# ReactiveBayes/RxInfer.jl

Measured on NVIDIA H100. Metric: gaussian_messages_per_sec_batched_lgssm_d4_T1000, higher is better.
Workload: dtype f32

## Files before the change

rxinfer.jl_b200/csrc/rxg_lgssm.cu:

```cuda
#include <math.h>
#include <stdlib.h>

#include <utility>

#include "rxg_chain_step.cuh"
#include "rxg_gain.cuh"
#include "rxg_internal.h"
#include "rxg_linalg.cuh"
#include "rxg_lgssm_cluster.cuh"
#include "rxg_lgssm_common.cuh"
#include "rxg_lgssm_shared.cuh"
#include "rxg_lgssm_seg.cuh"
#include "rxg_sweep_select.h"

namespace rxg {

template <int D, int M, bool PER_CHAIN, bool SMOOTH, bool USEQ = false>
__global__ void __launch_bounds__(128)
lgssm_chain_kernel(const __grid_constant__ ModelF<D, M> mdl, PerChainPtrs pc,
                   const float* __restrict__ y, const uint8_t* __restrict__ mask,
                   float* __restrict__ mean, float* __restrict__ cov, float* __restrict__ nle,
                   int32_t* __restrict__ status, int T, int64_t batch, int transition_first,
                   const float* __restrict__ useq = nullptr, int64_t ustride = 0, int uchain = 0) {
    const int64_t b = (int64_t)blockIdx.x * blockDim.x + threadIdx.x;
    if (b >= batch) return;

    Mat<float, D, D> A, P, S0;
    Mat<float, M, D> B;
    Mat<float, M, M> Q;
    Vec<float, D> mu, u;
    if (PER_CHAIN) {
        A = load_strided<float, D, D>(pc.A + b, batch);
        B = load_strided<float, M, D>(pc.B + b, batch);
        P = load_strided<float, D, D>(pc.P + b, batch);
        Q = load_strided<float, M, M>(pc.Q + b, batch);
        S0 = load_strided<float, D, D>(pc.S0 + b, batch);
#pragma unroll
        for (int i = 0; i < D; ++i) mu(i) = __ldg(pc.m0 + i * batch + b);
#pragma unroll
        for (int i = 0; i < D; ++i) u(i) = pc.u ? __ldg(pc.u + i * batch + b) : 0.f;
    } else {
        A = load_const<float, D, D>(mdl.A);
        B = load_const<float, M, D>(mdl.B);
        P = load_const<float, D, D>(mdl.P);
        Q = load_const<float, M, M>(mdl.Q);
        S0 = load_const<float, D, D>(mdl.S0);
#pragma unroll
        for (int i = 0; i < D; ++i) { mu(i) = mdl.m0[i]; u(i) = mdl.u[i]; }
    }
    Mat<float, D, D> S = S0;
    bool bad = false;
    double acc_nle = 0.0;
    const bool want_nle = (nle != nullptr);

    float ynext[M];
#pragma unroll
    for (int k = 0; k < M; ++k) ynext[k] = __ldg(y + (int64_t)k * batch + b);
    uint8_t onext = mask ? mask[b] : (uint8_t)1;

    for (int t = 0; t < T; ++t) {
        Vec<float, M> yt;
#pragma unroll
        for (int k = 0; k < M; ++k) yt(k) = ynext[k];
        const bool observed = onext != 0;
        if (t + 1 < T) {
#pragma unroll
            for (int k = 0; k < M; ++k) ynext[k] = __ldg(y + ((int64_t)(t + 1) * M + k) * batch + b);
            if (mask) onext = mask[(int64_t)(t + 1) * batch + b];
        }
        if (t > 0 || transition_first) {
            if constexpr (USEQ)
                chain_predict(A, P, u, [&](Vec<float, D>& uu) {
#pragma unroll
                    for (int i = 0; i < D; ++i) uu(i) = __ldg(useq + ((int64_t)t * D + i) * ustride + b * uchain);
                }, mu, S);
            else
                chain_predict(A, P, u, NoInput{}, mu, S);
        }
        if (observed) chain_update(B, Q, yt, want_nle, mu, S, bad, acc_nle);
#pragma unroll
        for (int i = 0; i < D; ++i) mean[((int64_t)t * D + i) * batch + b] = mu(i);
        const bool full = !SMOOTH || (t == T - 1);
#pragma unroll
        for (int i = 0; i < D; ++i)
#pragma unroll
            for (int j = 0; j < D; ++j)
                if (full || j <= i) cov[(((int64_t)t * D + i) * D + j) * batch + b] = S(i, j);
    }
    if (want_nle) nle[b] = (float)acc_nle;

    if (SMOOTH) {
        Vec<float, D> mus = mu;
        Mat<float, D, D> Ss = S;
        float pm[D], pS[D * (D + 1) / 2];
        if (T >= 2) {
            const int t = T - 2;
#pragma unroll
            for (int i = 0; i < D; ++i) pm[i] = mean[((int64_t)t * D + i) * batch + b];
            int q = 0;
#pragma unroll
            for (int i = 0; i < D; ++i)
#pragma unroll
                for (int j = 0; j <= i; ++j) pS[q++] = cov[(((int64_t)t * D + i) * D + j) * batch + b];
        }
        for (int t = T - 2; t >= 0; --t) {
            Vec<float, D> muf;
            Mat<float, D, D> Sf;
#pragma unroll
            for (int i = 0; i < D; ++i) muf(i) = pm[i];
            {
                int q = 0;
#pragma unroll
                for (int i = 0; i < D; ++i)
#pragma unroll
                    for (int j = 0; j <= i; ++j) { Sf(i, j) = pS[q]; Sf(j, i) = pS[q]; ++q; }
            }
            if (t > 0) {
                const int tp = t - 1;
#pragma unroll
                for (int i = 0; i < D; ++i) pm[i] = mean[((int64_t)tp * D + i) * batch + b];
                int q = 0;
#pragma unroll
                for (int i = 0; i < D; ++i)
#pragma unroll
                    for (int j = 0; j <= i; ++j) pS[q++] = cov[(((int64_t)tp * D + i) * D + j) * batch + b];
            }
            if constexpr (USEQ)
                chain_rts(A, P, u, [&](Vec<float, D>& uu) {
#pragma unroll
                    for (int i = 0; i < D; ++i) uu(i) = __ldg(useq + ((int64_t)(t + 1) * D + i) * ustride + b * uchain);
                }, muf, Sf, mus, Ss, bad);
            else
                chain_rts(A, P, u, NoInput{}, muf, Sf, mus, Ss, bad);
#pragma unroll
            for (int i = 0; i < D; ++i) mean[((int64_t)t * D + i) * batch + b] = mus(i);
#pragma unroll
            for (int i = 0; i < D; ++i)
#pragma unroll
                for (int j = 0; j < D; ++j) cov[(((int64_t)t * D + i) * D + j) * batch + b] = Ss(i, j);
        }
        mu = mus;
    }
    if (status) {
        bool nan = false;
#pragma unroll
        for (int i = 0; i < D; ++i) nan |= !(mu(i) == mu(i));
        status[b] = bad ? RXG_ERR_NOT_SPD : (nan ? RXG_ERR_NAN : RXG_OK);
    }
}

template <int D, int M>
__global__ void gain_riccati_seq(const __grid_constant__ ModelF<D, M> mdl, GainWs ws, int T,
                                 int transition_first, int* __restrict__ bad_out, const uint8_t* __restrict__ tmask) {
    if (threadIdx.x != 0 || blockIdx.x != 0) return;
    const Mat<double, D, D> A = load_const<double, D, D>(mdl.A), P = load_const<double, D, D>(mdl.P);
    const Mat<double, M, D> B = load_const<double, M, D>(mdl.B);
    const Mat<double, M, M> Q = load_const<double, M, M>(mdl.Q);
    Mat<double, D, D> S = load_const<double, D, D>(mdl.S0);
    bool bad = false;
    for (int t = 0; t < T; ++t) {
        if (t > 0 || transition_first) {
            Mat<double, D, D> AS = mul(A, S);
            S = sym_mul_nt_add(AS, A, P);
        }
        store_d(ws.Sp + (size_t)t * D * D, S);
        if (!tmask || tmask[t] != 0) {
            Mat<double, M, D> BS = mul(B, S);
            Mat<double, M, M> Sinn = sym_mul_nt_add(BS, B, Q);
            Chol<double, M> ch = cholesky<double, M, false>(Sinn, bad);
            Mat<double, D, M> V = solve_right_Lt(transpose(BS), ch.L);
            S = sym_downdate(S, V);
        }
        store_d(ws.Sf + (size_t)t * D * D, S);
    }
    if (bad) atomicOr(bad_out, 1);
}

template <int D, int M>
__global__ void gain_tables(const __grid_constant__ ModelF<D, M> mdl, GainWs ws, int T,
                            int transition_first, int* __restrict__ bad_out, const uint8_t* __restrict__ tmask,
                            const float* __restrict__ useq) {
    const int t = blockIdx.x * blockDim.x + threadIdx.x;
    if (t >= T) return;
    using TB = Tab<D, M>;
    const Mat<double, D, D> A = load_const<double, D, D>(mdl.A);
    const Mat<double, M, D> B = load_const<double, M, D>(mdl.B);
    const Mat<double, M, M> Q = load_const<double, M, M>(mdl.Q);
    bool bad = false;
    const Mat<double, D, D> Sp = load_d<D, D>(ws.Sp + (size_t)t * D * D);
    const Mat<double, D, D> Sf = load_d<D, D>(ws.Sf + (size_t)t * D * D);
    {
        Mat<double, D, M> K;
        Mat<double, M, M> Li;
        double cconst = 0.0;
#pragma unroll
        for (int i = 0; i < D * M; ++i) K.a[i] = 0.0;
#pragma unroll
        for (int i = 0; i < M * M; ++i) Li.a[i] = 0.0;
        if (!tmask || tmask[t] != 0) {
            Mat<double, M, D> BS = mul(B, Sp);
            Mat<double, M, M> Sinn = sym_mul_nt_add(BS, B, Q);
            Chol<double, M> ch = cholesky<double, M, true>(Sinn, bad);
            Mat<double, D, M> V = solve_right_Lt(transpose(BS), ch.L);
            K = solve_right_L(V, ch.L);
#pragma unroll
            for (int j = 0; j < M; ++j) {
                Li(j, j) = ch.L(j, j);
#pragma unroll
                for (int i = j + 1; i < M; ++i) {
                    double sacc = 0.0;
#pragma unroll
                    for (int k = j; k < i; ++k) sacc -= ch.L(i, k) * Li(k, j);
                    Li(i, j) = sacc * ch.L(i, i);
                }
            }
            cconst = M * RXG_HALF_LOG_2PI - ch.neg_half_logdet;
        }
        Mat<double, D, D> IKB = identity<double, D>();
#pragma unroll
        for (int i = 0; i < D; ++i)
#pragma unroll
            for (int j = 0; j < D; ++j)
#pragma unroll
                for (int k = 0; k < M; ++k) IKB(i, j) -= K(i, k) * B(k, j);
        Mat<double, D, D> F = (t > 0 || transition_first) ? mul(IKB, A) : IKB;
        float* rec = ws.fwd + (size_t)t * TB::FWD_REC;
        store_f(rec + TB::F_OFF, F);
        store_f(rec + TB::K_OFF, K);
        store_f(rec + TB::LI_OFF, Li);
        rec[TB::C_OFF] = (float)cconst;
        Vec<double, D> uu, gf;
#pragma unroll
        for (int i = 0; i < D; ++i) uu(i) = (double)(useq ? useq[(size_t)t * D + i] : mdl.u[i]);
        gf = mulv(IKB, uu);
        if (!(t > 0 || transition_first)) {
#pragma unroll
            for (int i = 0; i < D; ++i) gf(i) = 0.0;
        }
        store_fv(rec + TB::GF_OFF, gf);
        store_f(ws.sf + (size_t)t * TB::SF_REC, Sf);
    }
    float* brec = ws.bwd + (size_t)t * TB::BWD_REC;
    Vec<double, D> gb;
#pragma unroll
    for (int i = 0; i < D; ++i) gb(i) = 0.0;
    if (t < T - 1) {
        const Mat<double, D, D> Sp1 = load_d<D, D>(ws.Sp + (size_t)(t + 1) * D * D);
        Chol<double, D> ch = cholesky<double, D, false>(Sp1, bad);
        Mat<double, D, D> AS = mul(A, Sf);
        Mat<double, D, D> U = solve_right_Lt(transpose(AS), ch.L);
        Mat<double, D, D> G = solve_right_L(U, ch.L);
        Mat<double, D, D> C = sym_downdate(Sf, U);
        Mat<double, D, D> E = identity<double, D>();
        Mat<double, D, D> GA = mul(G, A);
#pragma unroll
        for (int i = 0; i < D * D; ++i) E.a[i] -= GA.a[i];
        store_f(brec + TB::E_OFF, E);
        store_f(brec + TB::G_OFF, G);
        {
            Vec<double, D> uu;
#pragma unroll
            for (int i = 0; i < D; ++i) uu(i) = -(double)(useq ? useq[(size_t)(t + 1) * D + i] : mdl.u[i]);
            gb = mulv(G, uu);
        }
        store_d(ws.Cc + (size_t)t * D * D, C);
        store_d(ws.Gd + (size_t)t * D * D, G);
    } else {
        Mat<double, D, D> E = identity<double, D>();
        Mat<double, D, D> Z;
#pragma unroll
        for (int i = 0; i < D * D; ++i) Z.a[i] = 0.0;
        store_f(brec + TB::E_OFF, E);
        store_f(brec + TB::G_OFF, Z);
    }
    store_fv(brec + TB::GB_OFF, gb);
    if (bad) atomicOr(bad_out, 1);
}

template <int D, int M>
__global__ void gain_smooth_seq(GainWs ws, int T, float* cov_shared_out) {
    if (threadIdx.x != 0 || blockIdx.x != 0) return;
    using TB = Tab<D, M>;
    Mat<double, D, D> Ss = load_d<D, D>(ws.Sf + (size_t)(T - 1) * D * D);
    store_f(ws.bwd + (size_t)(T - 1) * TB::BWD_REC + TB::SS_OFF, Ss);
    if (cov_shared_out) store_f(cov_shared_out + (size_t)(T - 1) * D * D, Ss);
    for (int t = T - 2; t >= 0; --t) {
        const Mat<double, D, D> G = load_d<D, D>(ws.Gd + (size_t)t * D * D);
        const Mat<double, D, D> C = load_d<D, D>(ws.Cc + (size_t)t * D * D);
        Mat<double, D, D> GS = mul(G, Ss);
        Ss = sym_mul_nt_add(GS, G, C);
        store_f(ws.bwd + (size_t)t * TB::BWD_REC + TB::SS_OFF, Ss);
        if (cov_shared_out) store_f(cov_shared_out + (size_t)t * D * D, Ss);
    }
}

static __global__ void copy_table_kernel(const float* __restrict__ tab, int rec, int n, int T, float* __restrict__ out) {
    const int i = blockIdx.x * blockDim.x + threadIdx.x;
    if (i < T * n) out[i] = tab[(size_t)(i / n) * rec + (i % n)];
}

template <int D, int M>
static void fill_model(ModelF<D, M>& mdl, const LgssmCall& c) {
    for (int i = 0; i < D * D; ++i) { mdl.A[i] = c.A[i]; mdl.P[i] = c.P[i]; mdl.S0[i] = c.S0[i]; }
    for (int i = 0; i < M * D; ++i) mdl.B[i] = c.B[i];
    for (int i = 0; i < M * M; ++i) mdl.Q[i] = c.Q[i];
    for (int i = 0; i < D; ++i) { mdl.m0[i] = c.m0[i]; mdl.u[i] = c.u ? c.u[i] : 0.f; }
}

template <int D, int M, bool PER_CHAIN, bool SMOOTH>
static void launch_chain(rxg_ctx* ctx, const LgssmCall& c, const ModelF<D, M>& mdl, const PerChainPtrs& pc) {
    const int threads = 64;
    const unsigned blocks = (unsigned)((c.batch + threads - 1) / threads);
    const int tf = (c.flags & RXG_TRANSITION_FIRST) ? 1 : 0;
    if (c.useq)
        lgssm_chain_kernel<D, M, PER_CHAIN, SMOOTH, true><<<blocks, threads, 0, ctx->stream>>>(
            mdl, pc, c.y, c.ymask, c.mean, c.cov, c.nle, c.status, c.T, c.batch, tf, c.useq, c.useq_chain ? c.batch : 1,
            c.useq_chain ? 1 : 0);
    else
        lgssm_chain_kernel<D, M, PER_CHAIN, SMOOTH><<<blocks, threads, 0, ctx->stream>>>(
            mdl, pc, c.y, c.ymask, c.mean, c.cov, c.nle, c.status, c.T, c.batch, tf);
}

template <int D, int M>
static int run_chain_family(rxg_ctx* ctx, LgssmCall& c) {
    ModelF<D, M> mdl = {};
    PerChainPtrs pc = {};
    const bool per_chain = (c.flags & RXG_MODEL_PER_CHAIN) != 0;
    if (per_chain) pc = PerChainPtrs{c.A, c.B, c.P, c.Q, c.m0, c.S0, c.u};
    else fill_model<D, M>(mdl, c);
    if (ctx->profile) { cudaEventRecord(ctx->ev[0], ctx->stream); cudaEventRecord(ctx->ev[1], ctx->stream); }
    if (per_chain) (c.smooth ? launch_chain<D, M, true, true> : launch_chain<D, M, true, false>)(ctx, c, mdl, pc);
    else           (c.smooth ? launch_chain<D, M, false, true> : launch_chain<D, M, false, false>)(ctx, c, mdl, pc);
    if (ctx->profile) cudaEventRecord(ctx->ev[2], ctx->stream);
    ctx->launches += 1;
    return check_cuda(ctx, cudaGetLastError(), "lgssm_chain_kernel launch");
}

template <int D, int M, int I>
static bool launch_sweep_if(int pick, rxg_ctx* ctx, const LgssmCall& c, const ModelF<D, M>& mdl, const GainWs& ws,
                            int write_cov) {
    constexpr SweepPick p = sweep_pick_at(I);
    if constexpr (sweep_pick_reachable(D, M, p)) {
        if (pick == I) {
            const int threads = 32;
            const unsigned blocks = (unsigned)((c.batch / p.cpt + threads - 1) / threads);
            const int tf = (c.flags & RXG_TRANSITION_FIRST) ? 1 : 0;
            lgssm_shared_kernel<D, M, p.cpt, 4, p.smooth, p.evid, p.offset, p.ckpt, p.peer, p.useq>
                <<<blocks, threads, 0, ctx->stream>>>(mdl, ws.fwd, ws.bwd, ws.sf, c.y, c.mean, c.cov, c.nle, c.T, c.batch,
                                                      tf, write_cov, c.mean0_chain, c.po, p.useq ? c.useq : nullptr);
            return true;
        }
    }
    return false;
}
template <int D, int M, int... I>
static bool launch_sweep(int pick, rxg_ctx* ctx, const LgssmCall& c, const ModelF<D, M>& mdl, const GainWs& ws,
                         int write_cov, std::integer_sequence<int, I...>) {
    return (launch_sweep_if<D, M, I>(pick, ctx, c, mdl, ws, write_cov) || ...);
}

template <int D, int M>
static int launch_shared(rxg_ctx* ctx, LgssmCall& c, const ModelF<D, M>& mdl, const GainWs& ws, int write_cov,
                         const SweepPick& p) {
    const int pick = sweep_pick_index(p);
    if (ctx->profile) cudaEventRecord(ctx->ev[1], ctx->stream);
    if (!launch_sweep<D, M>(pick, ctx, c, mdl, ws, write_cov, std::make_integer_sequence<int, SWEEP_PICK_COUNT>{}))
        return fail(ctx, RXG_ERR_UNSUPPORTED, "lgssm: no lgssm_shared_kernel instantiation for sweep pick %d", pick);
    if (ctx->profile) cudaEventRecord(ctx->ev[2], ctx->stream);
    ctx->launches += 1;
    c.fused_peer_stores = p.peer;
    return check_cuda(ctx, cudaGetLastError(), "lgssm_shared_kernel launch");
}

template <int D, int M>
static bool seg_sweep_eligible(const LgssmCall& c) {
    using ST = SegTab<D, M>;
    if (!c.smooth || c.nle || D * D > 16) return false;
    const int nseg = (c.T + ST::L - 1) / ST::L;
    const size_t smem = (size_t)nseg * 2 * D * 32 * 4 + (size_t)8 * 2 * ST::L * ST::REC * 4;
    return smem <= 200 * 1024;
}
template <int D, int M>
static int launch_seg(rxg_ctx* ctx, LgssmCall& c, const ModelF<D, M>& mdl, const GainWs& ws, const SegWs& sw, int write_cov,
                      bool hints) {
    using ST = SegTab<D, M>;
    constexpr int NW = 8;
    const int nseg = (c.T + ST::L - 1) / ST::L;
    seg_tables_kernel<D, M><<<(nseg + 63) / 64, 64, 0, ctx->stream>>>(ws, sw, c.T);
    const size_t smem = (size_t)nseg * 2 * D * 32 * 4 + (size_t)NW * 2 * ST::L * ST::REC * 4;
    const int64_t ntiles = (c.batch + 31) / 32;
    const unsigned grid = (unsigned)(ntiles < ctx->sm_count ? ntiles : ctx->sm_count);
    bool has_u = false;
    for (int i = 0; i < D; ++i) has_u |= (mdl.u[i] != 0.f);
#define RXG_LAUNCH_SEG(OF, HI)                                                                                        \
    do {                                                                                                               \
        RXG_CUDA(ctx, cudaFuncSetAttribute(lgssm_seg_kernel<D, M, NW, OF, HI>, cudaFuncAttributeMaxDynamicSharedMemorySize, (int)smem)); \
        if (ctx->profile) cudaEventRecord(ctx->ev[1], ctx->stream);                                                    \
        lgssm_seg_kernel<D, M, NW, OF, HI><<<grid, 32 * NW, smem, ctx->stream>>>(mdl, sw, c.y, c.mean, c.cov, c.T, c.batch, \
                                                                                 write_cov, c.mean0_chain, c.po, nseg);  \
    } while (0)
    (void)hints;
    if (has_u) RXG_LAUNCH_SEG(true, 1); else RXG_LAUNCH_SEG(false, 1);
#undef RXG_LAUNCH_SEG
    if (ctx->profile) cudaEventRecord(ctx->ev[2], ctx->stream);
    ctx->launches += 2;
    c.fused_peer_stores = false;
    return check_cuda(ctx, cudaGetLastError(), "lgssm_seg_kernel launch");
}

template <int D, int M>
static int launch_cluster_if_eligible(rxg_ctx* ctx, LgssmCall& c, const ModelF<D, M>& mdl, const GainWs& ws, float* cl_tab,
                                      int write_cov, bool& launched) {
    launched = false;
    if constexpr (D * D <= 16 && M >= D) {
        using CT = ClusterTab<D, M>;
        bool offset = false;
        for (int i = 0; i < D; ++i) offset |= (mdl.u[i] != 0.f);
        const bool aligned = (((uintptr_t)c.y | (uintptr_t)c.mean | (uintptr_t)c.cov) & 15) == 0;
        if (!c.smooth || c.nle || c.useq || offset || c.mean0_chain || c.batch % 32 != 0 || !aligned ||
            ctx->opt[RXG_OPT_SWEEP_VARIANT] != 0 || ctx->opt[RXG_OPT_FORCE_CPT] != 0)
            return RXG_OK;
        const size_t smem = CT::smem_bytes(c.T);
        int smem_max = 0;
        RXG_CUDA(ctx, cudaDeviceGetAttribute(&smem_max, cudaDevAttrMaxSharedMemoryPerBlockOptin, ctx->device));
        if (smem > (size_t)smem_max) return RXG_OK;
        const bool peer = c.po.n_mean > 0 || c.po.n_cov > 0;
        auto kern = peer ? lgssm_cluster_sweep_kernel<D, M, true> : lgssm_cluster_sweep_kernel<D, M, false>;
        RXG_CUDA(ctx, cudaFuncSetAttribute(kern, cudaFuncAttributeMaxDynamicSharedMemorySize, (int)smem));
        cudaLaunchConfig_t cfg = {};
        cudaLaunchAttribute attr[1];
        attr[0].id = cudaLaunchAttributeClusterDimension;
        attr[0].val.clusterDim.x = CL_CTAS;
        attr[0].val.clusterDim.y = 1;
        attr[0].val.clusterDim.z = 1;
        cfg.gridDim = dim3((unsigned)(c.batch / 32 * CL_CTAS));
        cfg.blockDim = dim3(32 * CL_WARPS);
        cfg.dynamicSmemBytes = smem;
        cfg.stream = ctx->stream;
        cfg.attrs = attr;
        cfg.numAttrs = 1;
        int nclusters = 0;
        RXG_CUDA(ctx, cudaOccupancyMaxActiveClusters(&nclusters, kern, &cfg));
        if (nclusters < 1) return RXG_OK;

        const int spc = CT::spc(c.T);
        cluster_tables_kernel<D, M><<<1, 256, 0, ctx->stream>>>(ws, cl_tab, c.T, spc);
        if (ctx->profile) cudaEventRecord(ctx->ev[1], ctx->stream);
        RXG_CUDA(ctx, cudaLaunchKernelEx(&cfg, kern, (const float*)ws.fwd, (const float*)ws.bwd, (const float*)cl_tab, c.y,
                                         c.mean, c.cov, c.T, c.batch, write_cov, mdl, c.po));
        if (ctx->profile) cudaEventRecord(ctx->ev[2], ctx->stream);
        ctx->launches += 2;
        c.fused_peer_stores = peer;
        launched = true;
        return check_cuda(ctx, cudaGetLastError(), "lgssm_cluster_sweep_kernel launch");
    }
    return RXG_OK;
}

template <int D, int M>
static int run_shared_family(rxg_ctx* ctx, LgssmCall& c) {
    using TB = Tab<D, M>;
    ModelF<D, M> mdl = {};
    fill_model<D, M>(mdl, c);
    const size_t T = (size_t)c.T;
    size_t off = 0;
    auto carve = [&](size_t bytes) { size_t o = off; off += (bytes + 255) / 256 * 256; return o; };
    const size_t o_fwd = carve(T * TB::FWD_REC * sizeof(float));
    const size_t o_bwd = carve(T * TB::BWD_REC * sizeof(float));
    const size_t o_sf = carve(T * TB::SF_REC * sizeof(float));
    const size_t o_Sp = carve(T * D * D * sizeof(double));
    const size_t o_Sf = carve(T * D * D * sizeof(double));
    const size_t o_Cc = carve(T * D * D * sizeof(double));
    const size_t o_Gd = carve(T * D * D * sizeof(double));
    const size_t o_fel = carve(T * 3 * D * D * sizeof(double));
    const size_t o_ftot = carve((size_t)2 * GS_NT * 3 * D * D * sizeof(double));
    const size_t o_bel = carve(T * 2 * D * D * sizeof(double));
    const size_t o_btot = carve((size_t)2 * GS_NT * 2 * D * D * sizeof(double));
    using ST = SegTab<D, M>;
    const size_t nseg = (T + ST::L - 1) / ST::L;
    const size_t o_srec_t = carve(T * ST::REC * sizeof(float)), o_snrec = carve(T * ST::NREC * sizeof(float));
    const size_t o_ssrec = carve(nseg * ST::SREC * sizeof(float));
    const size_t o_ctab = carve(c.want_cov_table ? T * D * D * sizeof(float) : 0);
    const size_t o_cl = carve(ClusterTab<D, M>::table_floats(c.T) * sizeof(float));
    char* base = (char*)workspace(ctx, off);
    if (!base) return RXG_ERR_CUDA;
    GainWs ws;
    ws.fwd = (float*)(base + o_fwd); ws.bwd = (float*)(base + o_bwd); ws.sf = (float*)(base + o_sf);
    ws.Sp = (double*)(base + o_Sp); ws.Sf = (double*)(base + o_Sf);
    ws.Cc = (double*)(base + o_Cc); ws.Gd = (double*)(base + o_Gd);
    ScanWs sw;
    sw.fel = (double*)(base + o_fel); sw.ftot = (double*)(base + o_ftot);
    sw.bel = (double*)(base + o_bel); sw.btot = (double*)(base + o_btot);

    const int tf = (c.flags & RXG_TRANSITION_FIRST) ? 1 : 0;
    const bool cov_shared = (c.flags & RXG_COV_SHARED_OUT) != 0;
    c.cov_table = (c.want_cov_table && c.smooth) ? (float*)(base + o_ctab) : nullptr;
    if (ctx->profile) cudaEventRecord(ctx->ev[0], ctx->stream);
    float* cov_once = (cov_shared && c.cov && c.smooth) ? c.cov : (c.smooth ? c.cov_table : nullptr);
    const float* useq_tab = c.useq_chain ? nullptr : c.useq;
    if (ctx->opt[RXG_OPT_GAIN_SEQ] != 0) {
        gain_riccati_seq<D, M><<<1, 32, 0, ctx->stream>>>(mdl, ws, c.T, tf, bad_flag(ctx), c.tmask);
        gain_tables<D, M><<<(c.T + 63) / 64, 64, 0, ctx->stream>>>(mdl, ws, c.T, tf, bad_flag(ctx), c.tmask, useq_tab);
        ctx->launches += 2;
        if (c.smooth) {
            gain_smooth_seq<D, M><<<1, 32, 0, ctx->stream>>>(ws, c.T, cov_once);
            ctx->launches += 1;
        }
    } else {
        gain_scan_kernel<D, M><<<GS_CTAS, GS_THREADS, 0, ctx->stream>>>(mdl, ws, sw, c.T, tf, cov_once, bad_flag(ctx), c.tmask,
                                                                          useq_tab);
        ctx->launches += 1;
    }
    if (!c.smooth && cov_shared && c.cov) {
        const int n = c.T * D * D;
        copy_table_kernel<<<(n + 255) / 256, 256, 0, ctx->stream>>>(ws.sf, TB::SF_REC, D * D, c.T, c.cov);
        ctx->launches += 1;
    }
    int rc = check_cuda(ctx, cudaGetLastError(), "gain table kernels launch");
    if (rc != RXG_OK) return rc;
    if (c.ev_tables) RXG_CUDA(ctx, cudaEventRecord(c.ev_tables, ctx->stream));
    if (c.tables_only) return RXG_OK;
    const int write_cov = (c.cov != nullptr && !cov_shared) ? 1 : 0;
    bool launched = false;
    rc = launch_cluster_if_eligible<D, M>(ctx, c, mdl, ws, (float*)(base + o_cl), write_cov, launched);
    if (rc != RXG_OK || launched) return rc;
    const long long variant = ctx->opt[RXG_OPT_SWEEP_VARIANT];
    if (variant == 3 && !c.useq && seg_sweep_eligible<D, M>(c)) {
        SegWs sgw;
        sgw.rec = (float*)(base + o_srec_t); sgw.nrec = (float*)(base + o_snrec); sgw.srec = (float*)(base + o_ssrec);
        return launch_seg<D, M>(ctx, c, mdl, ws, sgw, write_cov, variant == 3);
    }
    SweepQuery q = {};
    q.d = D;
    q.m = M;
    q.batch = c.batch;
    q.sm_count = ctx->sm_count;
    q.force_cpt = ctx->opt[RXG_OPT_FORCE_CPT];
    q.aligned16 = (((uintptr_t)c.y | (uintptr_t)c.mean | (uintptr_t)c.cov | (uintptr_t)c.nle | (uintptr_t)c.mean0_chain |
                    (uintptr_t)(c.useq_chain ? c.useq : nullptr)) & 15) == 0;
    q.smooth = c.smooth;
    q.evid = c.nle != nullptr;
    for (int i = 0; i < D; ++i) q.offset |= (mdl.u[i] != 0.f);
    q.input = !c.useq ? InputSeq::none : (c.useq_chain ? InputSeq::per_chain : InputSeq::shared);
    q.peer_out = c.po.n_mean > 0 || c.po.n_cov > 0;
    q.sweep_variant = variant;
    return launch_shared<D, M>(ctx, c, mdl, ws, write_cov, select_shared_sweep(q));
}

template <int D, int M>
int run_dm(rxg_ctx* ctx, LgssmCall& c) {
    const bool per_chain = (c.flags & (RXG_MODEL_PER_CHAIN | RXG_PATH_PER_CHAIN)) != 0 || c.ymask != nullptr;
    if (per_chain) return run_chain_family<D, M>(ctx, c);
    int rc = run_shared_family<D, M>(ctx, c);
    if (rc == RXG_OK && c.status) rc = fill_status_from_flag(ctx, c.status, c.batch);
    return rc;
}

#ifdef RXG_INST_D
template int run_dm<RXG_INST_D, RXG_INST_M>(rxg_ctx*, LgssmCall&);
#else
extern template int run_dm<1, 1>(rxg_ctx*, LgssmCall&);
extern template int run_dm<2, 1>(rxg_ctx*, LgssmCall&);
extern template int run_dm<2, 2>(rxg_ctx*, LgssmCall&);
extern template int run_dm<3, 3>(rxg_ctx*, LgssmCall&);
extern template int run_dm<4, 1>(rxg_ctx*, LgssmCall&);
extern template int run_dm<4, 2>(rxg_ctx*, LgssmCall&);
extern template int run_dm<4, 4>(rxg_ctx*, LgssmCall&);
extern template int run_dm<6, 6>(rxg_ctx*, LgssmCall&);

__global__ void fill_status_kernel(int32_t* s, int64_t n, const int* __restrict__ bad) {
    const int64_t i = (int64_t)blockIdx.x * blockDim.x + threadIdx.x;
    if (i < n) s[i] = (*bad != 0) ? (int32_t)RXG_ERR_NOT_SPD : (int32_t)RXG_OK;
}
int fill_status_from_flag(rxg_ctx* ctx, int32_t* status, int64_t n) {
    fill_status_kernel<<<(unsigned)((n + 255) / 256), 256, 0, ctx->stream>>>(status, n, bad_flag(ctx));
    ctx->launches += 1;
    return check_cuda(ctx, cudaGetLastError(), "fill_status launch");
}

int lgssm_dispatch_native(rxg_ctx* ctx, LgssmCall& c) {
    switch (c.d * 16 + c.m) {
        case 1 * 16 + 1: return run_dm<1, 1>(ctx, c);
        case 2 * 16 + 1: return run_dm<2, 1>(ctx, c);
        case 2 * 16 + 2: return run_dm<2, 2>(ctx, c);
        case 3 * 16 + 3: return run_dm<3, 3>(ctx, c);
        case 4 * 16 + 1: return run_dm<4, 1>(ctx, c);
        case 4 * 16 + 2: return run_dm<4, 2>(ctx, c);
        case 4 * 16 + 4: return run_dm<4, 4>(ctx, c);
        case 6 * 16 + 6: return run_dm<6, 6>(ctx, c);
        default:
            return fail(ctx, RXG_ERR_UNSUPPORTED,
                        "lgssm: (d=%d, m=%d) is outside the register-resident kernel families", c.d, c.m);
    }
}

#endif

}
```

rxinfer.jl_b200/csrc/rxg_lgssm_cluster.cuh:

```cuda
#pragma once
#include <cooperative_groups.h>

#include "rxg_lgssm_common.cuh"
#include "rxg_lgssm_shared.cuh"

namespace rxg {

constexpr int CL_CTAS = 8;
constexpr int CL_WARPS = 8;
constexpr int CL_L = 16;

template <int D, int M>
struct ClusterTab {
    static constexpr int FK = pad4(D * D) + pad4(D * M);
    static constexpr int EG = 2 * pad4(D * D);
    static constexpr int REC = 2 * pad4(D * D);
    static constexpr int PSI_OFF = pad4(D * D);
    static_assert(Tab<D, M>::F_OFF == 0 && Tab<D, M>::K_OFF == pad4(D * D) && Tab<D, M>::E_OFF == 0 &&
                      Tab<D, M>::G_OFF == pad4(D * D),
                  "the staged prefixes are the first FK / EG floats of the gain records");

    static __host__ __device__ int spc(int T) { return ((T + CL_L - 1) / CL_L + CL_CTAS - 1) / CL_CTAS; }
    static size_t table_floats(int T) { return (size_t)(CL_CTAS * spc(T) + CL_CTAS) * REC; }
    static size_t smem_bytes(int T) {
        const size_t S = (size_t)spc(T) * CL_L;
        return 4 * (S * (M * 32 + FK + EG) + (size_t)(spc(T) + CL_CTAS) * REC + (size_t)spc(T) * D * 32 + 2 * D * 32);
    }
};

template <int D, int M>
__global__ void __launch_bounds__(256) cluster_tables_kernel(GainWs ws, float* __restrict__ tab, int T, int spc) {
    using TB = Tab<D, M>;
    using CT = ClusterTab<D, M>;
    const int nsub = CL_CTAS * spc;
    for (int j = threadIdx.x; j < nsub; j += blockDim.x) {
        const int a = j * CL_L, e = min(a + CL_L, T);
        Mat<double, D, D> Phi = identity<double, D>(), Psi = identity<double, D>();
        for (int t = a; t < e; ++t) {
            Phi = mul(load_const<double, D, D>(ws.fwd + (size_t)t * TB::FWD_REC + TB::F_OFF), Phi);
            Psi = mul(Psi, load_const<double, D, D>(ws.bwd + (size_t)t * TB::BWD_REC + TB::G_OFF));
        }
        store_f(tab + (size_t)j * CT::REC, Phi);
        store_f(tab + (size_t)j * CT::REC + CT::PSI_OFF, Psi);
    }
    __syncthreads();
    for (int r = threadIdx.x; r < CL_CTAS; r += blockDim.x) {
        Mat<double, D, D> Phi = identity<double, D>(), Psi = identity<double, D>();
        for (int j = r * spc; j < (r + 1) * spc; ++j) {
            Phi = mul(load_const<double, D, D>(tab + (size_t)j * CT::REC), Phi);
            Psi = mul(Psi, load_const<double, D, D>(tab + (size_t)j * CT::REC + CT::PSI_OFF));
        }
        store_f(tab + (size_t)(nsub + r) * CT::REC, Phi);
        store_f(tab + (size_t)(nsub + r) * CT::REC + CT::PSI_OFF, Psi);
    }
}

template <int D>
__device__ __forceinline__ void affine_step(const float* Mx, float (&v)[D], const float (&w)[D]) {
    float Mr[pad4(D * D)];
    load_smem<pad4(D * D)>(Mx, Mr);
    float n[D];
#pragma unroll
    for (int i = 0; i < D; ++i) {
        float a = w[i];
#pragma unroll
        for (int j = 0; j < D; ++j) a = __fmaf_rn(Mr[i * D + j], v[j], a);
        n[i] = a;
    }
#pragma unroll
    for (int i = 0; i < D; ++i) v[i] = n[i];
}

template <int D, int M, bool PEER>
__global__ void __launch_bounds__(32 * CL_WARPS, 2)
lgssm_cluster_sweep_kernel(const float* __restrict__ fwd_tab, const float* __restrict__ bwd_tab,
                           const float* __restrict__ cl_tab, const float* __restrict__ y, float* __restrict__ mean,
                           float* __restrict__ cov, int T, int64_t batch, int write_cov,
                           const __grid_constant__ ModelF<D, M> mdl, const __grid_constant__ PeerOut po) {
    static_assert(M >= D, "pass B stores mu_f[t] over y_t");
    using TB = Tab<D, M>;
    using CT = ClusterTab<D, M>;
    namespace cg = cooperative_groups;
    cg::cluster_group cluster = cg::this_cluster();
    const int r = (int)cluster.block_rank();
    const int spc = CT::spc(T);
    const int S = spc * CL_L;
    const int t0 = r * S;
    const int nt = max(0, min(S, T - t0));
    const int warp = threadIdx.x >> 5, lane = threadIdx.x & 31;
    const int64_t b = ((int64_t)blockIdx.x / CL_CTAS) * 32 + lane;

    extern __shared__ __align__(16) float smem[];
    float* s_y = smem;
    float* s_fk = s_y + (size_t)S * M * 32;
    float* s_eg = s_fk + (size_t)S * CT::FK;
    float* s_sub = s_eg + (size_t)S * CT::EG;
    float* s_slice = s_sub + (size_t)spc * CT::REC;
    float* s_car = s_slice + CL_CTAS * CT::REC;
    float* s_off = s_car + (size_t)spc * D * 32;

    {
        const int tid = threadIdx.x;
        for (int p = tid; p < nt * M * 8; p += 32 * CL_WARPS) {
            const int row = p >> 3, part = p & 7;
            cp_async16(s_y + row * 32 + part * 4, y + ((int64_t)t0 * M + row) * batch + (b - lane) + part * 4);
        }
        for (int p = tid; p < nt * (CT::FK / 4); p += 32 * CL_WARPS) {
            const int s = p / (CT::FK / 4), part = p % (CT::FK / 4);
            cp_async16(s_fk + s * CT::FK + part * 4, fwd_tab + (size_t)(t0 + s) * TB::FWD_REC + part * 4);
        }
        for (int p = tid; p < nt * (CT::EG / 4); p += 32 * CL_WARPS) {
            const int s = p / (CT::EG / 4), part = p % (CT::EG / 4);
            cp_async16(s_eg + s * CT::EG + part * 4, bwd_tab + (size_t)(t0 + s) * TB::BWD_REC + part * 4);
        }
        for (int p = tid; p < spc * (CT::REC / 4); p += 32 * CL_WARPS)
            cp_async16(s_sub + p * 4, cl_tab + (size_t)r * spc * CT::REC + p * 4);
        for (int p = tid; p < CL_CTAS * (CT::REC / 4); p += 32 * CL_WARPS)
            cp_async16(s_slice + p * 4, cl_tab + (size_t)CL_CTAS * spc * CT::REC + p * 4);
        cp_async_commit();
        cp_async_wait<0>();
    }
    __syncthreads();

    auto car = [&](int j, int i) -> float& { return s_car[((size_t)j * D + i) * 32 + lane]; };
    auto off = [&](float* base, int dir, int i) -> float& { return base[(dir * D + i) * 32 + lane]; };

    for (int j = warp; j < spc; j += CL_WARPS) {
        float x[D];
#pragma unroll
        for (int i = 0; i < D; ++i) x[i] = 0.f;
#pragma unroll
        for (int q = 0; q < CL_L; ++q) {
            const int s = j * CL_L + q;
            if (s < nt) {
                float Ft[pad4(D * D)], Kt[pad4(D * M)];
                load_smem<pad4(D * D)>(s_fk + s * CT::FK, Ft);
                load_smem<pad4(D * M)>(s_fk + s * CT::FK + pad4(D * D), Kt);
                float nx[D];
#pragma unroll
                for (int i = 0; i < D; ++i) {
                    float a = Ft[i * D] * x[0];
#pragma unroll
                    for (int jj = 1; jj < D; ++jj) a = __fmaf_rn(Ft[i * D + jj], x[jj], a);
#pragma unroll
                    for (int k = 0; k < M; ++k) a = __fmaf_rn(Kt[i * M + k], s_y[(s * M + k) * 32 + lane], a);
                    nx[i] = a;
                }
#pragma unroll
                for (int i = 0; i < D; ++i) x[i] = nx[i];
            }
        }
#pragma unroll
        for (int i = 0; i < D; ++i) car(j, i) = x[i];
    }
    __syncthreads();

    if (warp == 0) {
        float z[D];
#pragma unroll
        for (int i = 0; i < D; ++i) z[i] = 0.f;
        for (int j = 0; j < spc; ++j) {
            float c[D];
#pragma unroll
            for (int i = 0; i < D; ++i) c[i] = car(j, i);
            affine_step<D>(s_sub + j * CT::REC, z, c);
        }
#pragma unroll
        for (int i = 0; i < D; ++i) off(s_off, 0, i) = z[i];
    }
    cluster.sync();
    if (warp == 0) {
        float x[D];
#pragma unroll
        for (int i = 0; i < D; ++i) x[i] = mdl.m0[i];
        for (int q = 0; q < r; ++q) {
            float* rem = cluster.map_shared_rank(s_off, q);
            float c[D];
#pragma unroll
            for (int i = 0; i < D; ++i) c[i] = off(rem, 0, i);
            affine_step<D>(s_slice + q * CT::REC, x, c);
        }
        for (int j = 0; j < spc; ++j) {
            float c[D];
#pragma unroll
            for (int i = 0; i < D; ++i) { c[i] = car(j, i); car(j, i) = x[i]; }
            affine_step<D>(s_sub + j * CT::REC, x, c);
        }
    }
    __syncthreads();

    for (int j = warp; j < spc; j += CL_WARPS) {
        float x[D];
#pragma unroll
        for (int i = 0; i < D; ++i) x[i] = car(j, i);
#pragma unroll
        for (int q = 0; q < CL_L; ++q) {
            const int s = j * CL_L + q;
            if (s < nt) {
                float Ft[pad4(D * D)], Kt[pad4(D * M)], yt[M];
                load_smem<pad4(D * D)>(s_fk + s * CT::FK, Ft);
                load_smem<pad4(D * M)>(s_fk + s * CT::FK + pad4(D * D), Kt);
#pragma unroll
                for (int k = 0; k < M; ++k) yt[k] = s_y[(s * M + k) * 32 + lane];
                float nx[D];
#pragma unroll
                for (int i = 0; i < D; ++i) {
                    float a = Ft[i * D] * x[0];
#pragma unroll
                    for (int jj = 1; jj < D; ++jj) a = __fmaf_rn(Ft[i * D + jj], x[jj], a);
#pragma unroll
                    for (int k = 0; k < M; ++k) a = __fmaf_rn(Kt[i * M + k], yt[k], a);
                    nx[i] = a;
                }
#pragma unroll
                for (int i = 0; i < D; ++i) { x[i] = nx[i]; s_y[(s * M + i) * 32 + lane] = nx[i]; }
            }
        }
        float v[D];
#pragma unroll
        for (int i = 0; i < D; ++i) v[i] = 0.f;
#pragma unroll
        for (int q = CL_L - 1; q >= 0; --q) {
            const int s = j * CL_L + q;
            if (s < nt) {
                float Et[pad4(D * D)], Gt[pad4(D * D)];
                load_smem<pad4(D * D)>(s_eg + s * CT::EG, Et);
                load_smem<pad4(D * D)>(s_eg + s * CT::EG + pad4(D * D), Gt);
                float nv[D];
#pragma unroll
                for (int i = 0; i < D; ++i) {
                    float a = Et[i * D] * s_y[(s * M) * 32 + lane];
#pragma unroll
                    for (int jj = 1; jj < D; ++jj) a = __fmaf_rn(Et[i * D + jj], s_y[(s * M + jj) * 32 + lane], a);
#pragma unroll
                    for (int jj = 0; jj < D; ++jj) a = __fmaf_rn(Gt[i * D + jj], v[jj], a);
                    nv[i] = a;
                }
#pragma unroll
                for (int i = 0; i < D; ++i) v[i] = nv[i];
            }
        }
#pragma unroll
        for (int i = 0; i < D; ++i) car(j, i) = v[i];
    }
    __syncthreads();

    if (warp == 0) {
        float z[D];
#pragma unroll
        for (int i = 0; i < D; ++i) z[i] = 0.f;
        for (int j = spc - 1; j >= 0; --j) {
            float c[D];
#pragma unroll
            for (int i = 0; i < D; ++i) c[i] = car(j, i);
            affine_step<D>(s_sub + j * CT::REC + CT::PSI_OFF, z, c);
        }
#pragma unroll
        for (int i = 0; i < D; ++i) off(s_off, 1, i) = z[i];
    }
    cluster.sync();
    if (warp == 0) {
        float v[D];
#pragma unroll
        for (int i = 0; i < D; ++i) v[i] = 0.f;
        for (int q = CL_CTAS - 1; q > r; --q) {
            float* rem = cluster.map_shared_rank(s_off, q);
            float c[D];
#pragma unroll
            for (int i = 0; i < D; ++i) c[i] = off(rem, 1, i);
            affine_step<D>(s_slice + q * CT::REC + CT::PSI_OFF, v, c);
        }
        for (int j = spc - 1; j >= 0; --j) {
            float c[D];
#pragma unroll
            for (int i = 0; i < D; ++i) { c[i] = car(j, i); car(j, i) = v[i]; }
            affine_step<D>(s_sub + j * CT::REC + CT::PSI_OFF, v, c);
        }
    }
    asm volatile("barrier.cluster.arrive.release.aligned;\n" ::: "memory");
    __syncthreads();

    for (int j = warp; j < spc; j += CL_WARPS) {
        float v[D][1];
#pragma unroll
        for (int i = 0; i < D; ++i) v[i][0] = car(j, i);
#pragma unroll
        for (int q = CL_L - 1; q >= 0; --q) {
            const int s = j * CL_L + q;
            if (s < nt) {
                const int t = t0 + s;
                float Et[pad4(D * D)], Gt[pad4(D * D)];
                load_smem<pad4(D * D)>(s_eg + s * CT::EG, Et);
                load_smem<pad4(D * D)>(s_eg + s * CT::EG + pad4(D * D), Gt);
                float nv[D];
#pragma unroll
                for (int i = 0; i < D; ++i) {
                    float a = Et[i * D] * s_y[(s * M) * 32 + lane];
#pragma unroll
                    for (int jj = 1; jj < D; ++jj) a = __fmaf_rn(Et[i * D + jj], s_y[(s * M + jj) * 32 + lane], a);
#pragma unroll
                    for (int jj = 0; jj < D; ++jj) a = __fmaf_rn(Gt[i * D + jj], v[jj][0], a);
                    nv[i] = a;
                }
#pragma unroll
                for (int i = 0; i < D; ++i) {
                    v[i][0] = nv[i];
                    __stcs(mean + ((int64_t)t * D + i) * batch + b, nv[i]);
                }
                float Sst[pad4(D * D)];
                if (write_cov) {
                    load_uniform<pad4(D * D)>(bwd_tab + (size_t)t * TB::BWD_REC + TB::SS_OFF, Sst);
#pragma unroll
                    for (int i = 0; i < D * D; ++i) __stcs(cov + ((int64_t)t * D * D + i) * batch + b, Sst[i]);
                }
                if (PEER) peer_store<D, 1>(po, write_cov, t, batch, b, v, Sst);
            }
        }
    }
    asm volatile("barrier.cluster.wait.acquire.aligned;\n" ::: "memory");
}

}
```

rxinfer.jl_b200/csrc/rxg_umma.cuh:

```cuda
#pragma once
#include <cuda_runtime.h>
#include <stdint.h>

namespace rxg {
namespace umma {

constexpr uint32_t LBO = 128;
__host__ __device__ constexpr uint32_t sbo_bytes(int K) { return (uint32_t)(K / 4) * 128u; }
__host__ __device__ constexpr uint32_t elem_off(int row, int k, int K) {
    return (uint32_t)(row / 8) * sbo_bytes(K) + (uint32_t)(k / 4) * LBO + (uint32_t)(row % 8) * 16u + (uint32_t)(k % 4) * 4u;
}

__device__ __forceinline__ uint64_t smem_desc(uint32_t smem_addr, uint32_t lbo, uint32_t sbo) {
    uint64_t d = 0;
    d |= (uint64_t)((smem_addr >> 4) & 0x3FFF);
    d |= (uint64_t)((lbo >> 4) & 0x3FFF) << 16;
    d |= (uint64_t)((sbo >> 4) & 0x3FFF) << 32;
    return d;
}

template <int N>
__device__ __forceinline__ void mma_tf32(float* d, uint64_t adesc, uint64_t bdesc, uint32_t accumulate);

template <>
__device__ __forceinline__ void mma_tf32<16>(float* d, uint64_t adesc, uint64_t bdesc, uint32_t accumulate) {
    asm volatile(
        "{\n\t"
        ".reg .pred p;\n\t"
        "setp.ne.b32 p, %10, 0;\n\t"
        "wgmma.mma_async.sync.aligned.m64n16k8.f32.tf32.tf32 "
        "{%0, %1, %2, %3, %4, %5, %6, %7}, %8, %9, p, 1, 1;\n\t"
        "}\n"
        : "+f"(d[0]), "+f"(d[1]), "+f"(d[2]), "+f"(d[3]), "+f"(d[4]), "+f"(d[5]), "+f"(d[6]), "+f"(d[7])
        : "l"(adesc), "l"(bdesc), "r"(accumulate));
}

template <>
__device__ __forceinline__ void mma_tf32<32>(float* d, uint64_t adesc, uint64_t bdesc, uint32_t accumulate) {
    asm volatile(
        "{\n\t"
        ".reg .pred p;\n\t"
        "setp.ne.b32 p, %18, 0;\n\t"
        "wgmma.mma_async.sync.aligned.m64n32k8.f32.tf32.tf32 "
        "{%0, %1, %2, %3, %4, %5, %6, %7, %8, %9, %10, %11, %12, %13, %14, %15}, %16, %17, p, 1, 1;\n\t"
        "}\n"
        : "+f"(d[0]), "+f"(d[1]), "+f"(d[2]), "+f"(d[3]), "+f"(d[4]), "+f"(d[5]), "+f"(d[6]), "+f"(d[7]),
          "+f"(d[8]), "+f"(d[9]), "+f"(d[10]), "+f"(d[11]), "+f"(d[12]), "+f"(d[13]), "+f"(d[14]), "+f"(d[15])
        : "l"(adesc), "l"(bdesc), "r"(accumulate));
}

__device__ __forceinline__ void wgmma_fence() { asm volatile("wgmma.fence.sync.aligned;" ::: "memory"); }
__device__ __forceinline__ void wgmma_commit() { asm volatile("wgmma.commit_group.sync.aligned;" ::: "memory"); }
__device__ __forceinline__ void wgmma_wait_all() { asm volatile("wgmma.wait_group.sync.aligned 0;" ::: "memory"); }
__device__ __forceinline__ void fence_reg(float& r) { asm volatile("" : "+f"(r)::"memory"); }
__device__ __forceinline__ void fence_async_smem() { asm volatile("fence.proxy.async.shared::cta;" ::: "memory"); }

__device__ __forceinline__ void mbar_init(uint64_t* mbar, uint32_t count) {
    asm volatile("mbarrier.init.shared::cta.b64 [%0], %1;" ::"r"((uint32_t)__cvta_generic_to_shared(mbar)), "r"(count) : "memory");
}

__device__ __forceinline__ void mbar_expect_tx(uint64_t* mbar, uint32_t bytes) {
    asm volatile("mbarrier.arrive.expect_tx.shared::cta.b64 _, [%0], %1;" ::"r"((uint32_t)__cvta_generic_to_shared(mbar)),
                 "r"(bytes)
                 : "memory");
}
__device__ __forceinline__ void bulk_g2s(void* smem_dst, const void* gmem_src, uint32_t bytes, uint64_t* mbar) {
    asm volatile("cp.async.bulk.shared::cluster.global.mbarrier::complete_tx::bytes [%0], [%1], %2, [%3];" ::"r"(
                     (uint32_t)__cvta_generic_to_shared(smem_dst)),
                 "l"(gmem_src), "r"(bytes), "r"((uint32_t)__cvta_generic_to_shared(mbar))
                 : "memory");
}
__device__ __forceinline__ void mbar_wait_bounded(uint64_t* mbar, uint32_t parity) {
    const uint32_t a = (uint32_t)__cvta_generic_to_shared(mbar);
    uint32_t done = 0;
    for (uint32_t spin = 0; spin < (1u << 27); ++spin) {
        asm volatile(
            "{\n\t"
            ".reg .pred p;\n\t"
            "mbarrier.try_wait.parity.shared::cta.b64 p, [%1], %2;\n\t"
            "selp.u32 %0, 1, 0, p;\n\t"
            "}\n"
            : "=r"(done)
            : "r"(a), "r"(parity)
            : "memory");
        if (done) return;
    }
    __trap();
}

__device__ __forceinline__ void split_tf32(float x, float& hi, float& lo) {
    uint32_t h;
    asm("cvt.rna.tf32.f32 %0, %1;" : "=r"(h) : "f"(x));
    hi = __uint_as_float(h);
    const float r = x - hi;
    uint32_t l;
    asm("cvt.rna.tf32.f32 %0, %1;" : "=r"(l) : "f"(r));
    lo = __uint_as_float(l);
}

}
}
```

Baseline: 144.2 billion.

## Offload covariance stores to a dedicated producer warp using bulk smem-to-global copies

Adds a ninth warp per CTA that writes the batch-uniform smoothed covariance output. It fills a shared staging buffer and issues cp.async.bulk shared-to-global copies with an L2 evict-first hint, paced against the cluster barriers. The compute warps no longer issue per-element streaming stores of the covariance and synchronise among themselves with a named barrier. This overlaps the dominant covariance write traffic with the recursion, at the cost of an extra warp, more shared memory and more intricate barrier coordination.

New measurement: 152.1 billion (median of 6 runs). 1.06x the previous value.

```diff
diff --git a/rxinfer.jl_b200/csrc/rxg_lgssm.cu b/rxinfer.jl_b200/csrc/rxg_lgssm.cu
--- a/rxinfer.jl_b200/csrc/rxg_lgssm.cu
+++ b/rxinfer.jl_b200/csrc/rxg_lgssm.cu
@@ -434,7 +434,7 @@
         attr[0].val.clusterDim.y = 1;
         attr[0].val.clusterDim.z = 1;
         cfg.gridDim = dim3((unsigned)(c.batch / 32 * CL_CTAS));
-        cfg.blockDim = dim3(32 * CL_WARPS);
+        cfg.blockDim = dim3(CL_THREADS);
         cfg.dynamicSmemBytes = smem;
         cfg.stream = ctx->stream;
         cfg.attrs = attr;
diff --git a/rxinfer.jl_b200/csrc/rxg_lgssm_cluster.cuh b/rxinfer.jl_b200/csrc/rxg_lgssm_cluster.cuh
--- a/rxinfer.jl_b200/csrc/rxg_lgssm_cluster.cuh
+++ b/rxinfer.jl_b200/csrc/rxg_lgssm_cluster.cuh
@@ -3,11 +3,14 @@
 
 #include "rxg_lgssm_common.cuh"
 #include "rxg_lgssm_shared.cuh"
+#include "rxg_umma.cuh"
 
 namespace rxg {
 
 constexpr int CL_CTAS = 8;
 constexpr int CL_WARPS = 8;
+constexpr int CL_THREADS = 32 * (CL_WARPS + 1);
+constexpr int CL_CS_LINES = 16;
 constexpr int CL_L = 16;
 
 template <int D, int M>
@@ -21,10 +24,12 @@
                   "the staged prefixes are the first FK / EG floats of the gain records");
 
     static __host__ __device__ int spc(int T) { return ((T + CL_L - 1) / CL_L + CL_CTAS - 1) / CL_CTAS; }
+    static __host__ __device__ int64_t cov_line(int64_t g, int T) { return g * T * (D * D) / CL_CTAS; }
     static size_t table_floats(int T) { return (size_t)(CL_CTAS * spc(T) + CL_CTAS) * REC; }
     static size_t smem_bytes(int T) {
         const size_t S = (size_t)spc(T) * CL_L;
-        return 4 * (S * (M * 32 + FK + EG) + (size_t)(spc(T) + CL_CTAS) * REC + (size_t)spc(T) * D * 32 + 2 * D * 32);
+        return 4 * (S * (M * 32 + FK + EG) + (size_t)(spc(T) + CL_CTAS) * REC + (size_t)spc(T) * D * 32 + 2 * D * 32 +
+                    CL_CS_LINES * 32);
     }
 };
 
@@ -71,8 +76,42 @@
     for (int i = 0; i < D; ++i) v[i] = n[i];
 }
 
+template <int D, int M>
+__device__ __forceinline__ void cov_write(const float* __restrict__ bwd_tab, float* __restrict__ cov, int64_t a,
+                                          int64_t e, int R, float* buf, int lane, int64_t& held) {
+    using TB = Tab<D, M>;
+    int64_t row = a / R;
+    int in = (int)(a - row * R);
+    for (int64_t l = a; l < e;) {
+        const int np = e - l < CL_CS_LINES ? (int)(e - l) : CL_CS_LINES;
+        const bool one = in + np <= R;
+        if (!one || row != held) {
+            if (lane == 0) umma::bulk_wait_read_all();
+            __syncwarp();
+#pragma unroll 4
+            for (int k = 0; k < CL_CS_LINES; ++k) {
+                const int64_t rw = row + (in + min(k, np - 1)) / R;
+                buf[k * 32 + lane] = __ldg(bwd_tab + rw / (D * D) * TB::BWD_REC + TB::SS_OFF + rw % (D * D));
+            }
+            umma::fence_async_smem();
+            __syncwarp();
+            held = one ? row : -1;
+        }
+        if (lane == 0) {
+            umma::bulk_s2g(cov + l * 32, buf, np * 128, umma::l2_evict_first_policy());
+            umma::bulk_commit();
+        }
+        l += np;
+        in += np;
+        row += in / R;
+        in %= R;
+    }
+}
+
+__device__ __forceinline__ void bar_rec() { asm volatile("bar.sync 1, %0;" ::"n"(32 * CL_WARPS) : "memory"); }
+
 template <int D, int M, bool PEER>
-__global__ void __launch_bounds__(32 * CL_WARPS, 2)
+__global__ void __launch_bounds__(CL_THREADS, 2)
 lgssm_cluster_sweep_kernel(const float* __restrict__ fwd_tab, const float* __restrict__ bwd_tab,
                            const float* __restrict__ cl_tab, const float* __restrict__ y, float* __restrict__ mean,
                            float* __restrict__ cov, int T, int64_t batch, int write_cov,
@@ -98,6 +137,27 @@
     float* s_slice = s_sub + (size_t)spc * CT::REC;
     float* s_car = s_slice + CL_CTAS * CT::REC;
     float* s_off = s_car + (size_t)spc * D * 32;
+    float* s_cs = s_off + 2 * D * 32;
+
+    if (warp == CL_WARPS) {
+        const int64_t c0 = CT::cov_line(blockIdx.x, T), c1 = CT::cov_line((int64_t)blockIdx.x + 1, T);
+        const int64_t cut1 = c0 + (c1 - c0) * 2 / 5, cut2 = c0 + (c1 - c0) * 4 / 5;
+        const int R = (int)(batch / 32);
+        int64_t held = -1;
+        asm volatile("barrier.cluster.arrive.release.aligned;\n" ::: "memory");
+        if (write_cov) cov_write<D, M>(bwd_tab, cov, c0, cut1, R, s_cs, lane, held);
+        asm volatile("barrier.cluster.wait.acquire.aligned;\n" ::: "memory");
+        asm volatile("barrier.cluster.arrive.release.aligned;\n" ::: "memory");
+        if (write_cov) cov_write<D, M>(bwd_tab, cov, cut1, cut2, R, s_cs, lane, held);
+        asm volatile("barrier.cluster.wait.acquire.aligned;\n" ::: "memory");
+        asm volatile("barrier.cluster.arrive.release.aligned;\n" ::: "memory");
+        if (write_cov) {
+            cov_write<D, M>(bwd_tab, cov, cut2, c1, R, s_cs, lane, held);
+            if (lane == 0) umma::bulk_wait_all();
+        }
+        asm volatile("barrier.cluster.wait.acquire.aligned;\n" ::: "memory");
+        return;
+    }
 
     {
         const int tid = threadIdx.x;
@@ -120,7 +180,7 @@
         cp_async_commit();
         cp_async_wait<0>();
     }
-    __syncthreads();
+    bar_rec();
 
     auto car = [&](int j, int i) -> float& { return s_car[((size_t)j * D + i) * 32 + lane]; };
     auto off = [&](float* base, int dir, int i) -> float& { return base[(dir * D + i) * 32 + lane]; };
@@ -153,7 +213,7 @@
 #pragma unroll
         for (int i = 0; i < D; ++i) car(j, i) = x[i];
     }
-    __syncthreads();
+    bar_rec();
 
     if (warp == 0) {
         float z[D];
@@ -187,7 +247,7 @@
             affine_step<D>(s_sub + j * CT::REC, x, c);
         }
     }
-    __syncthreads();
+    bar_rec();
 
     for (int j = warp; j < spc; j += CL_WARPS) {
         float x[D];
@@ -243,7 +303,7 @@
 #pragma unroll
         for (int i = 0; i < D; ++i) car(j, i) = v[i];
     }
-    __syncthreads();
+    bar_rec();
 
     if (warp == 0) {
         float z[D];
@@ -278,7 +338,7 @@
         }
     }
     asm volatile("barrier.cluster.arrive.release.aligned;\n" ::: "memory");
-    __syncthreads();
+    bar_rec();
 
     for (int j = warp; j < spc; j += CL_WARPS) {
         float v[D][1];
@@ -307,13 +367,11 @@
                     v[i][0] = nv[i];
                     __stcs(mean + ((int64_t)t * D + i) * batch + b, nv[i]);
                 }
-                float Sst[pad4(D * D)];
-                if (write_cov) {
-                    load_uniform<pad4(D * D)>(bwd_tab + (size_t)t * TB::BWD_REC + TB::SS_OFF, Sst);
-#pragma unroll
-                    for (int i = 0; i < D * D; ++i) __stcs(cov + ((int64_t)t * D * D + i) * batch + b, Sst[i]);
-                }
-                if (PEER) peer_store<D, 1>(po, write_cov, t, batch, b, v, Sst);
+                if (PEER) {
+                    float Sst[pad4(D * D)];
+                    if (write_cov) load_uniform<pad4(D * D)>(bwd_tab + (size_t)t * TB::BWD_REC + TB::SS_OFF, Sst);
+                    peer_store<D, 1>(po, write_cov, t, batch, b, v, Sst);
+                }
             }
         }
     }
diff --git a/rxinfer.jl_b200/csrc/rxg_umma.cuh b/rxinfer.jl_b200/csrc/rxg_umma.cuh
--- a/rxinfer.jl_b200/csrc/rxg_umma.cuh
+++ b/rxinfer.jl_b200/csrc/rxg_umma.cuh
@@ -70,6 +70,20 @@
                  "l"(gmem_src), "r"(bytes), "r"((uint32_t)__cvta_generic_to_shared(mbar))
                  : "memory");
 }
+__device__ __forceinline__ uint64_t l2_evict_first_policy() {
+    uint64_t pol;
+    asm volatile("createpolicy.fractional.L2::evict_first.b64 %0, 1.0;" : "=l"(pol));
+    return pol;
+}
+__device__ __forceinline__ void bulk_s2g(void* gmem_dst, const void* smem_src, uint32_t bytes, uint64_t pol) {
+    asm volatile("cp.async.bulk.global.shared::cta.bulk_group.L2::cache_hint [%0], [%1], %2, %3;" ::"l"(gmem_dst),
+                 "r"((uint32_t)__cvta_generic_to_shared(smem_src)), "r"(bytes), "l"(pol)
+                 : "memory");
+}
+__device__ __forceinline__ void bulk_commit() { asm volatile("cp.async.bulk.commit_group;" ::: "memory"); }
+__device__ __forceinline__ void bulk_wait_read_all() { asm volatile("cp.async.bulk.wait_group.read 0;" ::: "memory"); }
+__device__ __forceinline__ void bulk_wait_all() { asm volatile("cp.async.bulk.wait_group 0;" ::: "memory"); }
+
 __device__ __forceinline__ void mbar_wait_bounded(uint64_t* mbar, uint32_t parity) {
     const uint32_t a = (uint32_t)__cvta_generic_to_shared(mbar);
     uint32_t done = 0;
```
